# frosinastojanovska/image-captioning

Hardware: AMD Instinct MI355X
Metric: captions/sec (train step) on 1024px x 32RoI x 15tok synth (higher is better)
Workload: dtype f32 (split-bf16x3 products, fp32 accumulate: 73 of 85 conv layers on the bf16 pipe, the rest and the decoder exact fp32 MFMA); 1 GPU; BASELINE configs[2] (configs[3] at 8 GPUs): frozen ResNet-101+FPN fwd + PyramidROIAlign + RoI head + v2-inject decoder fwd/bwd + AMSGrad, 1024x1024 synth images, 32 RoI/img, 15-token captions, V=10000; backbone=resnet101, images_per_gpu=2, global_batch_images=2, parallelism=dp1, stage4_blocks=22, pipeline=encoder(i+1) || decoder(i), 2 HIP streams, rccl_ranks=1

## Files before the change

image-captioning_amd/_lib.py:

```python
import ctypes as C
import os

_HERE = os.path.dirname(os.path.abspath(__file__))
LIB_PATH = os.path.join(_HERE, "csrc", "libdcap_hip.so")

c_float_p = C.POINTER(C.c_float)
c_int32_p = C.POINTER(C.c_int32)
c_uint8_p = C.POINTER(C.c_uint8)


class GemmDesc(C.Structure):
    _fields_ = [("M", C.c_int), ("N", C.c_int), ("K", C.c_int),
                ("A", C.c_void_p), ("lda", C.c_int), ("a_trans", C.c_int),
                ("a_gather", C.c_void_p),
                ("B", C.c_void_p), ("ldb", C.c_int), ("b_trans", C.c_int),
                ("C", C.c_void_p), ("ldc", C.c_int),
                ("scale", C.c_void_p), ("shift", C.c_void_p),
                ("residual", C.c_void_p), ("ldr", C.c_int), ("res_rows", C.c_int),
                ("relu", C.c_int), ("accumulate", C.c_int), ("split_k", C.c_int)]


class GemmBf16Desc(C.Structure):
    _fields_ = [("M", C.c_int), ("N", C.c_int), ("K", C.c_int),
                ("A", C.c_void_p), ("lda", C.c_int), ("a_trans", C.c_int),
# ... 169 lines not shown


class DetectionTargetsDesc(C.Structure):
    _fields_ = [("n_proposals", C.c_int), ("n_gt", C.c_int), ("n_rois", C.c_int), ("T", C.c_int),
                ("proposals", C.c_void_p), ("gt_boxes", C.c_void_p), ("gt_captions", C.c_void_p),
                ("max_positive", C.c_int), ("inv_ratio", C.c_float), ("shuffle", C.c_int),
                ("seed", C.c_uint32), ("offset", C.c_uint32), ("offset_dev", C.c_void_p),
                ("rois", C.c_void_p), ("captions", C.c_void_p), ("counts", C.c_void_p)]


class PwChainDesc(C.Structure):
    _fields_ = [("M", C.c_int), ("K1", C.c_int), ("N1", C.c_int), ("N2", C.c_int),
                ("x", C.c_void_p), ("w1", C.c_void_p), ("scale1", C.c_void_p), ("shift1", C.c_void_p), ("residual", C.c_void_p),
                ("relu1", C.c_int), ("y", C.c_void_p), ("w2", C.c_void_p), ("scale2", C.c_void_p), ("shift2", C.c_void_p),
                ("relu2", C.c_int), ("z", C.c_void_p), ("w1_b3", C.c_void_p), ("w2_b3", C.c_void_p)]


class RegSegments(C.Structure):
    _fields_ = [("start", C.c_void_p), ("coef", C.c_void_p), ("mask", C.c_void_p), ("nseg", C.c_int)]


class AmsgradDesc(C.Structure):
    _fields_ = [("n", C.c_size_t), ("p", C.c_void_p), ("g", C.c_void_p), ("m", C.c_void_p),
                ("v", C.c_void_p), ("vhat", C.c_void_p),
                ("lr_t", C.c_float), ("beta1", C.c_float), ("beta2", C.c_float), ("eps", C.c_float),
                ("grad_scale", C.c_float), ("gnorm_sq", C.c_void_p), ("clipnorm", C.c_float),
                ("p_bf16", C.c_void_p), ("n_bf16", C.c_size_t), ("lr_t_dev", C.c_void_p), ("reg", C.POINTER(RegSegments))]


SYMBOLS = {
# ... 13 lines not shown
    "dc_cast_f32_bf16": (C.c_int, [C.c_void_p, C.c_void_p, C.c_size_t, C.c_void_p]),
    "dc_cast_bf16_f32": (C.c_int, [C.c_void_p, C.c_void_p, C.c_size_t, C.c_void_p]),
    "dc_cast_f32_bf16_2d": (C.c_int, [C.c_void_p, C.c_int, C.c_void_p, C.c_int, C.c_int, C.c_int, C.c_int, C.c_void_p]),
    "dc_split_bf16x3_f32": (C.c_int, [C.c_void_p, C.c_void_p, C.c_size_t, C.c_void_p]),
    "dc_conv2d_workspace_bytes": (C.c_size_t, [C.POINTER(ConvDesc)]),
    "dc_conv2d_nhwc_f32": (C.c_int, [C.POINTER(ConvDesc), C.c_void_p, C.c_size_t, C.c_void_p]),
    "dc_conv2d_tile_config": (C.c_int, [C.POINTER(ConvDesc), C.POINTER(C.c_int), C.POINTER(C.c_int), C.POINTER(C.c_int)]),
    "dc_conv2d_is_pointwise": (C.c_int, [C.POINTER(ConvDesc)]),
    "dc_conv2d_winograd_weight_bytes": (C.c_size_t, [C.c_int, C.c_int]),
    "dc_conv2d_winograd_pack_f32": (C.c_int, [C.c_void_p, C.c_void_p, C.c_int, C.c_int, C.c_void_p]),
    "dc_pw_chain_supported": (C.c_int, [C.c_int, C.c_int, C.c_int]),
    "dc_pw_chain_pack_f32": (C.c_int, [C.c_void_p, C.c_void_p, C.c_int, C.c_int, C.c_void_p]),
    "dc_pw_chain_pack_b3": (C.c_int, [C.c_void_p, C.c_void_p, C.c_int, C.c_int, C.c_void_p]),
    "dc_pw_chain_f32": (C.c_int, [C.POINTER(PwChainDesc), C.c_void_p]),
    "dc_pw_chain_kernel_name": (C.c_int, [C.POINTER(PwChainDesc), C.c_char_p, C.c_size_t]),
    "dc_conv2d_winograd_b3_weight_bytes": (C.c_size_t, [C.c_int, C.c_int]),
    "dc_conv2d_winograd_pack_b3": (C.c_int, [C.c_void_p, C.c_void_p, C.c_int, C.c_int, C.c_void_p]),
    "dc_conv2d_kernel_name": (C.c_int, [C.POINTER(ConvDesc), C.c_char_p, C.c_size_t]),
    "dc_conv2d_wgrad_workspace_bytes": (C.c_size_t, [C.POINTER(ConvDesc)]),
    "dc_conv2d_wgrad_f32": (C.c_int, [C.POINTER(ConvDesc), C.c_void_p, C.c_size_t, C.c_void_p]),
    "dc_roi_align_pyramid_bwd_f32": (C.c_int, [C.POINTER(RoiAlignDesc), C.c_void_p]),
    "dc_downsample2x_sum_f32": (C.c_int, [C.c_void_p, C.c_void_p, C.c_int, C.c_int, C.c_int, C.c_int, C.c_int, C.c_void_p]),
    "dc_downsample2x_sum_dual_f32": (C.c_int, [C.c_void_p, C.c_void_p, C.c_void_p, C.c_int, C.c_int, C.c_int, C.c_int, C.c_int, C.c_void_p]),
    "dc_maxpool2x2s2_f32": (C.c_int, [C.c_void_p, C.c_void_p, C.c_int, C.c_int, C.c_int, C.c_int, C.c_void_p]),
    "dc_maxpool3x3s2_same_f32": (C.c_int, [C.c_void_p, C.c_void_p, C.c_int, C.c_int, C.c_int, C.c_int, C.c_void_p]),
    "dc_mold_image_padded_f32": (C.c_int, [C.c_void_p, C.c_void_p, C.c_int, C.c_int, C.c_int, C.c_int, C.c_float, C.c_float, C.c_float, C.c_void_p]),
    "dc_mold_image_rgbx_f32": (C.c_int, [C.c_void_p, C.c_void_p, C.c_int, C.c_int, C.c_int,
                                         C.c_float, C.c_float, C.c_float, C.c_void_p]),
    "dc_roi_align_pyramid_f32": (C.c_int, [C.POINTER(RoiAlignDesc), C.c_void_p]),
    "dc_roi_tile_groups": (C.c_int, [C.POINTER(RoiGroupsDesc), C.c_void_p]),
# ... 102 lines not shown
```

image-captioning_amd/csrc/conv_chain.hip:

```cpp
#include "igemm_bf16s.h"
#include <algorithm>

namespace dcap {
namespace chain {

struct Args {
    const float* x;
    const f4* w1;
    const float* scale1;
    const float* shift1;
    const float* residual;
    float* y;
    const f4* w2;
    const float* scale2;
    const float* shift2;
    float* z;
    int M, K1, relu1, relu2;
    unsigned w1_bytes, w2_bytes;
};

__global__ void chain_pack_kernel(const float* __restrict__ w, float* __restrict__ out, int N, int K) {
    const long total = (long)N * K;
    const int NG = K >> 3;
    for (long idx = (long)blockIdx.x * blockDim.x + threadIdx.x; idx < total; idx += (long)gridDim.x * blockDim.x) {
        const int cout = (int)(idx / K), k = (int)(idx - (long)cout * K);
        const int cb = cout >> 5, i = cout & 31, g = k >> 3, h = (k >> 2) & 1, e = k & 3;
        out[(((long)cb * NG + g) * 64 + (h * 32 + i)) * 4 + e] = w[idx];
    }
}

__global__ void chain_pack_b3_kernel(const float* __restrict__ w, unsigned short* __restrict__ out, int N, int K) {
    const long total = (long)N * K;
    const int NG = K >> 4;
// ... 222 lines not shown
    }
    }
    if (m0 + p < a.M) {
#pragma unroll
        for (int gq = 0; gq < 4; ++gq) {
            const int c0 = wave * 32 + 8 * gq + 4 * h;
            f4 v = {acc2[4 * gq], acc2[4 * gq + 1], acc2[4 * gq + 2], acc2[4 * gq + 3]};
            if (a.scale2) v = v * *reinterpret_cast<const f4*>(a.scale2 + c0);
            v = v + *reinterpret_cast<const f4*>(a.shift2 + c0);
            if (a.relu2) v = f4{fmaxf(v[0], 0.f), fmaxf(v[1], 0.f), fmaxf(v[2], 0.f), fmaxf(v[3], 0.f)};
            *reinterpret_cast<f4*>(a.z + (long)(m0 + p) * N2 + c0) = v;
        }
    }
}

template <int K1, int N1, int N2>
__global__ __launch_bounds__(512, 1) void pw_chain_stream_kernel(Args a) {
    extern __shared__ __attribute__((aligned(16))) float smem[];
    constexpr int LDW1 = K1 + 4, LDW2 = N1 + 4, KH = K1 / 2, NG1 = K1 / 8, NG2 = N1 / 8;
    float* const W1s = smem;
    float* const W2s = W1s + N1 * LDW1;
    float* const sc1 = W2s + N2 * LDW2;
    float* const sh1 = sc1 + N1;
    float* const sc2 = sh1 + N1;
    float* const sh2 = sc2 + N2;
    const int tid = threadIdx.x, lane = tid & 63, wave = tid >> 6;
    const int i = lane & 31, h = lane >> 5;
    for (int idx = tid; idx < N1 * (K1 / 4); idx += 512) {
        const int c = idx / (K1 / 4), k4 = idx - c * (K1 / 4);
        *reinterpret_cast<f4*>(&W1s[c * LDW1 + 4 * k4]) = a.w1[((c >> 5) * NG1 + (k4 >> 1)) * 64 + 32 * (k4 & 1) + (c & 31)];
    }
    for (int idx = tid; idx < N2 * (N1 / 4); idx += 512) {
        const int c = idx / (N1 / 4), k4 = idx - c * (N1 / 4);
        *reinterpret_cast<f4*>(&W2s[c * LDW2 + 4 * k4]) = a.w2[((c >> 5) * NG2 + (k4 >> 1)) * 64 + 32 * (k4 & 1) + (c & 31)];
    }
    for (int c = tid; c < N1; c += 512) {
        sc1[c] = a.scale1 ? a.scale1[c] : 1.f;
        sh1[c] = a.shift1[c];
    }
    for (int c = tid; c < N2; c += 512) {
        sc2[c] = a.scale2 ? a.scale2[c] : 1.f;
        sh2[c] = a.shift2[c];
    }
    __syncthreads();
    const int strips = (a.M + 31) / 32;
    for (int st = blockIdx.x * 8 + wave; st < strips; st += gridDim.x * 8) {
        const int prow = st * 32 + i;
        const bool pv = prow < a.M;
        const int p = min(prow, a.M - 1);
        const float* xr = a.x + (long)p * K1 + KH * h;
        f4 xs[KH / 4];
#pragma unroll
        for (int j = 0; j < KH / 4; ++j) xs[j] = *reinterpret_cast<const f4*>(xr + 4 * j);
        const float* rrow = a.residual ? a.residual + (long)p * N1 + 4 * h : nullptr;
        float* const yrow = a.y + (long)p * N1 + 4 * h;
        f32x16 acc2[N2 / 32];
#pragma unroll
        for (int nb = 0; nb < N2 / 32; ++nb)
#pragma unroll
            for (int r = 0; r < 16; ++r) acc2[nb][r] = 0.f;
        for (int cb = 0; cb < N1; cb += 64) {
            f4 r0[4], r1[4];
            if (rrow) {
#pragma unroll
                for (int q = 0; q < 4; ++q) {
                    r0[q] = *reinterpret_cast<const f4*>(rrow + cb + 8 * q);
                    r1[q] = *reinterpret_cast<const f4*>(rrow + cb + 32 + 8 * q);
                }
            }
            f32x16 acc0, acc1;
#pragma unroll
            for (int r = 0; r < 16; ++r) { acc0[r] = 0.f; acc1[r] = 0.f; }
            const float* wa0 = &W1s[(cb + i) * LDW1 + KH * h];
            const float* wa1 = wa0 + 32 * LDW1;
#pragma unroll
            for (int j = 0; j < KH / 4; ++j) {
                const f4 a0 = *reinterpret_cast<const f4*>(wa0 + 4 * j);
                const f4 a1 = *reinterpret_cast<const f4*>(wa1 + 4 * j);
                const f4 b = xs[j];
#pragma unroll
                for (int e = 0; e < 4; ++e) {
                    acc0 = __builtin_amdgcn_mfma_f32_32x32x2f32(a0[e], b[e], acc0, 0, 0, 0);
                    acc1 = __builtin_amdgcn_mfma_f32_32x32x2f32(a1[e], b[e], acc1, 0, 0, 0);
                }
            }
            f4 y0[4], y1[4];
#pragma unroll
            for (int q = 0; q < 4; ++q) {
                const int c0 = cb + 8 * q + 4 * h;
                f4 v0 = f4{acc0[4 * q], acc0[4 * q + 1], acc0[4 * q + 2], acc0[4 * q + 3]} * *reinterpret_cast<const f4*>(&sc1[c0]) + *reinterpret_cast<const f4*>(&sh1[c0]);
                f4 v1 = f4{acc1[4 * q], acc1[4 * q + 1], acc1[4 * q + 2], acc1[4 * q + 3]} * *reinterpret_cast<const f4*>(&sc1[c0 + 32]) +
                        *reinterpret_cast<const f4*>(&sh1[c0 + 32]);
                if (rrow) { v0 += r0[q]; v1 += r1[q]; }
                if (a.relu1) {
                    v0 = f4{fmaxf(v0[0], 0.f), fmaxf(v0[1], 0.f), fmaxf(v0[2], 0.f), fmaxf(v0[3], 0.f)};
                    v1 = f4{fmaxf(v1[0], 0.f), fmaxf(v1[1], 0.f), fmaxf(v1[2], 0.f), fmaxf(v1[3], 0.f)};
                }
                if (pv) {
                    *reinterpret_cast<f4*>(yrow + cb + 8 * q) = v0;
                    *reinterpret_cast<f4*>(yrow + cb + 32 + 8 * q) = v1;
                }
                y0[q] = v0;
                y1[q] = v1;
            }
#pragma unroll
            for (int q = 0; q < 4; ++q)
#pragma unroll
                for (int nb = 0; nb < N2 / 32; ++nb) {
                    const float* w2r = &W2s[(nb * 32 + i) * LDW2 + cb + 8 * q + 4 * h];
                    const f4 wa = *reinterpret_cast<const f4*>(w2r);
                    const f4 wb = *reinterpret_cast<const f4*>(w2r + 32);
#pragma unroll
                    for (int e = 0; e < 4; ++e) {
                        acc2[nb] = __builtin_amdgcn_mfma_f32_32x32x2f32(wa[e], y0[q][e], acc2[nb], 0, 0, 0);
                        acc2[nb] = __builtin_amdgcn_mfma_f32_32x32x2f32(wb[e], y1[q][e], acc2[nb], 0, 0, 0);
                    }
                }
        }
// ... 1 lines not shown
            float* const zrow = a.z + (long)p * N2 + 4 * h;
#pragma unroll
            for (int nb = 0; nb < N2 / 32; ++nb)
#pragma unroll
                for (int q = 0; q < 4; ++q) {
                    const int c0 = nb * 32 + 8 * q + 4 * h;
                    f4 v = f4{acc2[nb][4 * q], acc2[nb][4 * q + 1], acc2[nb][4 * q + 2], acc2[nb][4 * q + 3]} * *reinterpret_cast<const f4*>(&sc2[c0]) +
                           *reinterpret_cast<const f4*>(&sh2[c0]);
                    if (a.relu2) v = f4{fmaxf(v[0], 0.f), fmaxf(v[1], 0.f), fmaxf(v[2], 0.f), fmaxf(v[3], 0.f)};
                    *reinterpret_cast<f4*>(zrow + nb * 32 + 8 * q) = v;
                }
        }
    }
}

static int launch_stream_64_256_64(const Args& a, hipStream_t s) {
    constexpr int K1 = 64, N1 = 256, N2 = 64;
    constexpr size_t lds = ((size_t)N1 * (K1 + 4) + (size_t)N2 * (N1 + 4) + 2 * N1 + 2 * N2) * sizeof(float);
    DC_ENSURE_DYN_LDS((&pw_chain_stream_kernel<K1, N1, N2>), 160 * 1024);
    const int strips = (a.M + 31) / 32;
    const int grid = std::max(1, std::min(kNumCU, (strips + 7) / 8));
    hipLaunchKernelGGL((pw_chain_stream_kernel<K1, N1, N2>), dim3(grid), dim3(512), lds, s, a);
    return check_launch("pw_chain_stream_kernel");
}

template <int CB1, int NB2, bool B3>
static int launch(const Args& a, hipStream_t s) {
    constexpr size_t lds = (size_t)32 * (CB1 * 256 + 4) * sizeof(float);
    DC_ENSURE_DYN_LDS((&pw_chain_kernel<CB1, NB2, B3>), 160 * 1024);
    hipLaunchKernelGGL((pw_chain_kernel<CB1, NB2, B3>), dim3((a.M + 31) / 32), dim3(512), lds, s, a);
    return check_launch("pw_chain_kernel");
}

}
}

using namespace dcap;

// ... 28 lines not shown
extern "C" int dc_pw_chain_f32(const dc_pw_chain_desc* d, void* stream) {
    const bool b3 = d && d->w1_b3 && d->w2_b3;
    DC_REQUIRE(d && d->x && (b3 || (d->w1 && d->w2)) && d->shift1 && d->y && d->shift2 && d->z && d->M > 0, DC_EINVAL, "dc_pw_chain: bad arguments");
    DC_REQUIRE(dc_pw_chain_supported(d->K1, d->N1, d->N2), DC_EINVAL,
               "dc_pw_chain: (K1, N1, N2) = (%d, %d, %d) is not a covered shape (K1 %% 32 == 0; N1 -> N2 = 1024 -> 256 or 512 -> 128; or 64 -> 256 -> 64)", d->K1, d->N1, d->N2);
    DC_REQUIRE(d->N1 != 256 || !b3, DC_EINVAL, "dc_pw_chain: the 64 -> 256 -> 64 seam takes fp32 products (dc_pw_chain_pack_f32 weights)");
    DC_REQUIRE(aligned16(d->x) && aligned16(b3 ? (const void*)d->w1_b3 : (const void*)d->w1) && aligned16(b3 ? (const void*)d->w2_b3 : (const void*)d->w2) && aligned16(d->y) && aligned16(d->z) && aligned16(d->shift1) && aligned16(d->shift2) &&
                   (!d->scale1 || aligned16(d->scale1)) && (!d->scale2 || aligned16(d->scale2)) && (!d->residual || aligned16(d->residual)),
               DC_EALIGN, "dc_pw_chain: every pointer must be 16-byte aligned");
    chain::Args a;
    a.x = d->x; a.w1 = b3 ? reinterpret_cast<const f4*>(d->w1_b3) : reinterpret_cast<const f4*>(d->w1); a.scale1 = d->scale1; a.shift1 = d->shift1; a.residual = d->residual; a.y = d->y;
    a.w2 = b3 ? reinterpret_cast<const f4*>(d->w2_b3) : reinterpret_cast<const f4*>(d->w2); a.scale2 = d->scale2; a.shift2 = d->shift2; a.z = d->z;
    a.M = d->M; a.K1 = d->K1; a.relu1 = d->relu1; a.relu2 = d->relu2;
    a.w1_bytes = (unsigned)((size_t)d->N1 * d->K1 * (b3 ? 6 : 4));
    a.w2_bytes = (unsigned)((size_t)d->N2 * d->N1 * (b3 ? 6 : 4));
    hipStream_t s = static_cast<hipStream_t>(stream);
    if (d->N1 == 256) return chain::launch_stream_64_256_64(a, s);
    if (b3) return d->N1 == 1024 ? chain::launch<4, 8, true>(a, s) : chain::launch<2, 4, true>(a, s);
    return d->N1 == 1024 ? chain::launch<4, 8, false>(a, s) : chain::launch<2, 4, false>(a, s);
}
```

image-captioning_amd/encoder.py:

```python
import ctypes as C

import numpy as np
import torch

from . import _lib, ops, step_graph
from ._lib import ConvBf16Desc, ConvDesc, PwChainDesc, check
from .layers import ConvSpec, resnet_fpn_convs
from .packing import fold_bn, pack_conv_kernel, pack_stem_kernel


DEFAULT_CONV_MATH = "f32"


def conv_math_mode(math=None):
    import os
    name = math if math is not None else os.environ.get("DCAP_CONV_MATH", DEFAULT_CONV_MATH)
    try:
        return {"f32": _lib.MATH_F32, "bf16x3": _lib.MATH_BF16X3, "bf16x2": _lib.MATH_BF16X2, "bf16": _lib.MATH_BF16}[name]
    except KeyError:
        raise ValueError("conv math must be 'f32', 'bf16x3', 'bf16x2' or 'bf16', got %r" % (name,))


def conv_math_name(mode):
    return {_lib.MATH_F32: "f32", _lib.MATH_BF16X3: "bf16x3", _lib.MATH_BF16X2: "bf16x2", _lib.MATH_BF16: "bf16"}.get(mode, str(mode))
# ... 5 lines not shown
    pad = (channels or k.shape[3]) - k.shape[3]
    if pad < 0:
        raise ValueError("rpn head needs %d channels, got %d" % (k.shape[3], channels))
    if pad:
        k = np.concatenate([k, np.zeros(k.shape[:3] + (pad,), np.float32)], axis=3)
        b = np.concatenate([b, np.zeros(pad, np.float32)])
    return k, b


class EncoderPlan:
    feat_channels = 256
    fast_bf16 = False

    def __init__(self, weights, batch, height, width, device, stage4_blocks=22,
                 mean_pixel=(123.7, 116.8, 103.9), use_graph=True, rpn=None, external=None, math=None, external_bn=None, train_stages=(),
                 winograd=None, wino_products=None, pw_chain=None, layer_math=None):
        if height % 64 or width % 64:
            raise ValueError("Image size must be dividable by 2 at least 6 times (got %dx%d)" % (height, width))
        self.lib = _lib.load()
        self.math = conv_math_mode(math)
        import os
        self.fast_bf16 = self.math == _lib.MATH_BF16
        self.winograd = (os.environ.get("DCAP_WINOGRAD", "1") != "0") if winograd is None else bool(winograd)
        self.wino_products = wino_products or os.environ.get("DCAP_WINO_PRODUCTS", "b3")
        if self.wino_products not in ("b3", "f32"):
            raise ValueError("wino_products must be 'b3' or 'f32'")
        self.pw_chain = (os.environ.get("DCAP_PW_CHAIN", "1") != "0") if pw_chain is None else bool(pw_chain)
        self.layer_math = (os.environ.get("DCAP_LAYER_MATH", "1") != "0") if layer_math is None else bool(layer_math)
        self._wchain = {}
        self._wwino = {}
        self._twin = {}
        self._wb = {}
        self.B, self.H, self.W = batch, height, width
        self.device = torch.device(device)
        self.mean_pixel = [float(v) for v in mean_pixel]
        self.stage4_blocks = stage4_blocks
        self.use_graph = bool(use_graph)
        self._steps = {}
        self._specs = {s.name: s for s in resnet_fpn_convs(stage4_blocks)}
        self.rpn = rpn
        self._external = dict(external or {})
        self._external_bn = dict(external_bn or {})
# ... 125 lines not shown
        if s.k != 1:
            return self.math
        if s.stride == 2 and s.cout >= 512 and s.cout > s.cin:
            return _lib.MATH_BF16X3
        if s.stride == 1 and 128 <= s.cin <= 512 and s.cout >= 256:
            return _lib.MATH_BF16X3
        return self.math

    def _chain_ok(self, name_c, name_a, mid, cout, pixels):
        sc, sa = self._specs[name_c], self._specs[name_a]
        if cout >= 512 and pixels < 32 * 192:
            return False
        return (self.pw_chain and self.math == _lib.MATH_F32 and not self.fast_bf16 and sc.k == 1 and sa.k == 1 and sc.stride == 1 and sa.stride == 1
                and name_c not in self._external and name_a not in self._external and ops.pw_chain_supported(mid, cout, mid))

    def _chain(self, name_c, x, y, residual, name_a, z):
        (w1, sc1, sh1), (w2, sc2, sh2) = self._w[name_c], self._w[name_a]
        b3 = self.wino_products == "b3" and x.shape[3] >= 128
        for n, w in ((name_c, w1), (name_a, w2)):
            if n not in self._wchain:
                self._wchain[n] = (ops.pw_chain_pack_b3 if b3 else ops.pw_chain_pack)(w)
        N, H, W, K1 = x.shape
        d = PwChainDesc()
        d.M, d.K1, d.N1, d.N2 = N * H * W, K1, y.shape[3], z.shape[3]
        d.x, d.shift1, d.y = x.data_ptr(), sh1.data_ptr(), y.data_ptr()
        if b3:
            d.w1_b3, d.w2_b3 = self._wchain[name_c].data_ptr(), self._wchain[name_a].data_ptr()
        else:
            d.w1, d.w2 = self._wchain[name_c].data_ptr(), self._wchain[name_a].data_ptr()
        d.scale1 = None if sc1 is None else sc1.data_ptr()
        d.residual = None if residual is None else residual.data_ptr()
        d.shift2, d.z = sh2.data_ptr(), z.data_ptr()
        d.scale2 = None if sc2 is None else sc2.data_ptr()
        d.relu1 = d.relu2 = 1
        self._ops.append(("chain", d, name_c + "+" + name_a))
        self.flops += 2.0 * d.M * (d.K1 * d.N1 + d.N1 * d.N2)

    def _build(self):
        B, H, W = self.B, self.H, self.W
        self._ops, self._ws_bytes, self.flops, self._bufs = [], 0, 0.0, []
        self._twin, self._wb = {}, {}
        self.images = torch.empty((B, H, W, 3), dtype=torch.uint8, device=self.device)
        rgbx = torch.empty((B, H, W, 4), dtype=torch.float32, device=self.device)
        for name, bnp in self._external_bn.items():
            _, sc, sh = self._external[name]
            self._ops.append(("bnfold", bnp, sc, sh))
        self._ops.append(("mold", self.images, rgbx))
        c1 = self._buf(H // 2, W // 2, 64)
        self._conv("conv1", rgbx, c1)
        x = self._buf(H // 4, W // 4, 64)
        self._ops.append(("pool", c1, x))
        if self.fast_bf16:
            self._ops.append(("cast", x, self._bf(x)))
        self.saved[1] = dict(rgbx=rgbx, c1=c1, pooled=x)

        def stage(s, blocks, mid, cout, stride, x):
            h, w = x.shape[1] // stride, x.shape[2] // stride
            keep = s in self.train_stages
            if not keep:
                m1, m2, sc = self._buf(h, w, mid), self._buf(h, w, mid), self._buf(h, w, cout)
                pp = [self._buf(h, w, cout), self._buf(h, w, cout)]
            final = self._buf(h, w, cout)
            self.saved[s] = []
            pending = None
            for i, blk in enumerate(blocks):
                cn = "res%d%s_branch" % (s, blk)
                if keep:
                    m1, m2 = self._buf(h, w, mid), self._buf(h, w, mid)
                    sc = self._buf(h, w, cout) if i == 0 else None
                    out = final if i == len(blocks) - 1 else self._buf(h, w, cout)
                    self.saved[s].append(dict(name=cn, x=x, m1=m1, m2=m2, sc=sc, out=out, stride=stride if i == 0 else 1))
                else:
                    out = final if i == len(blocks) - 1 else pp[i & 1]
                if pending is not None:
                    self._chain(pending[0], pending[1], x, pending[2], cn + "2a", m1)
                    pending = None
                else:
                    self._conv(cn + "2a", x, m1, f32=keep, bf16=True)
                self._conv(cn + "2b", m1, m2, f32=keep, bf16=True)
                res = x
                if i == 0:
                    self._conv(cn + "1", x, sc, relu=False)
                    res = sc
                nxt = "res%d%s_branch2a" % (s, blocks[i + 1]) if i + 1 < len(blocks) else None
                if nxt is not None and not keep and self._chain_ok(cn + "2c", nxt, mid, cout, x.shape[0] * m2.shape[1] * m2.shape[2]):
                    pending = (cn + "2c", m2, res)
                else:
                    self._conv(cn + "2c", m2, out, residual=res, res_mode=1, bf16=True)
                x = out
            return x

        C2 = stage(2, "abc", 64, 256, 1, x)
        C3 = stage(3, "abcd", 128, 512, 2, C2)
        C4 = stage(4, ["a"] + [chr(98 + i) for i in range(self.stage4_blocks)], 256, 1024, 2, C3)
        C5 = stage(5, "abc", 512, 2048, 2, C4)
        self.C = (C2, C3, C4, C5)
        self._n_trunk = len(self._ops)
        self.pre = None
        t5, t4 = self._buf(H // 32, W // 32, 256), self._buf(H // 16, W // 16, 256)
        t3, t2 = self._buf(H // 8, W // 8, 256), self._buf(H // 4, W // 4, 256)
        self._conv("fpn_c5p5", C5, t5, relu=False, bf16=True)
# ... 47 lines not shown

    def _run_ops(self, lo=0, hi=None):
        lib = self.lib
        stream = C.c_void_p(torch.cuda.current_stream().cuda_stream)
        wsp, wsb = C.c_void_p(self._ws.data_ptr()), self._ws.numel()
        for op in self._ops[lo:hi]:
            kind = op[0]
            if kind == "conv":
                rc = lib.dc_conv2d_nhwc_f32(C.byref(op[1]), wsp, wsb, stream)
                if rc:
                    check(rc, "dc_conv2d_nhwc_f32(%s)" % op[2])
            elif kind == "chain":
                rc = lib.dc_pw_chain_f32(C.byref(op[1]), stream)
                if rc:
                    check(rc, "dc_pw_chain_f32(%s)" % op[2])
            elif kind == "bconv":
                rc = lib.dc_conv2d_bf16(C.byref(op[1]), wsp, wsb, stream)
                if rc:
                    check(rc, "dc_conv2d_bf16(%s)" % op[2])
            elif kind == "cast":
                ops.to_bf16(op[1], out=op[2])
            elif kind == "bnfold":
                b = op[1]
                ops.bn_fold(b["gamma"], b["beta"], b["bias"], b["mean"], b["var"], op[2], op[3])
            elif kind == "mold":
                ops.mold_image_rgbx(op[1], self.mean_pixel, out=op[2])
            elif kind == "sub2":
                ops.subsample2(op[1], out=op[2])
            else:
                ops.maxpool3x3s2_same(op[1], out=op[2])

    def conv_table(self):
        rows = []
        for op in self._ops:
            if op[0] == "chain":
                d, buf = op[1], C.create_string_buffer(64)
                check(self.lib.dc_pw_chain_kernel_name(C.byref(d), buf, 64), "dc_pw_chain_kernel_name")
                rows.append((op[2], 2.0 * d.M * (d.K1 * d.N1 + d.N1 * d.N2), 32, d.N1, 1, buf.value.decode()))
                continue
            if op[0] != "conv":
                continue
            d, bm, bn, sk = op[1], C.c_int(), C.c_int(), C.c_int()
            check(self.lib.dc_conv2d_tile_config(C.byref(d), C.byref(bm), C.byref(bn), C.byref(sk)), "dc_conv2d_tile_config")
            buf = C.create_string_buffer(128)
            check(self.lib.dc_conv2d_kernel_name(C.byref(d), buf, 128), "dc_conv2d_kernel_name")
            s = self._specs[op[2]]
            rows.append((op[2], 2.0 * d.N * d.Ho * d.Wo * d.Cout * s.k * s.k * s.cin, bm.value, bn.value, sk.value, buf.value.decode()))
        return rows

    def conv_algorithmic_bytes(self):
        out = {}
        for op in self._ops:
            if op[0] == "chain":
                d = op[1]
                out[op[2]] = 4.0 * (d.M * (d.K1 + (2 if d.residual else 1) * d.N1 + d.N2) + d.K1 * d.N1 + d.N1 * d.N2)
                continue
            if op[0] != "conv":
                continue
            d, s = op[1], self._specs[op[2]]
            wbytes = ((16 * (6 if self.wino_products == "b3" else 4)) if op[2] in self._wwino else s.k * s.k * 4) * d.Cin * s.cout
            b = 4.0 * d.N * d.H * d.W * d.Cin + 4.0 * d.N * d.Ho * d.Wo * d.Cout + wbytes
            if d.res_mode == 1:
                b += 4.0 * d.N * d.Ho * d.Wo * d.Cout
            elif d.res_mode == 2:
                b += 1.0 * d.N * d.Ho * d.Wo * d.Cout
            out[op[2]] = b
        return out

    def time_convs(self, reps=3, beside=None):
        lib = self.lib
        stream = C.c_void_p(torch.cuda.current_stream().cuda_stream)
        wsp, wsb = C.c_void_p(self._ws.data_ptr()), self._ws.numel()
        convs = [op for op in self._ops if op[0] in ("conv", "chain")]
        acc = [0.0] * len(convs)
        for _ in range(reps):
            self._run_ops()
            torch.cuda.synchronize()
            if beside is not None:
                beside()
            evs = []
            for op in convs:
                e0, e1 = torch.cuda.Event(enable_timing=True), torch.cuda.Event(enable_timing=True)
                e0.record()
                rc = lib.dc_pw_chain_f32(C.byref(op[1]), stream) if op[0] == "chain" else lib.dc_conv2d_nhwc_f32(C.byref(op[1]), wsp, wsb, stream)
                e1.record()
                if rc:
                    check(rc, "dc_conv2d_nhwc_f32(%s)" % op[2])
                evs.append((e0, e1))
            torch.cuda.synchronize()
            for i, (e0, e1) in enumerate(evs):
                acc[i] += e0.elapsed_time(e1)
        return [(op[2], a / reps) for op, a in zip(convs, acc)]

    def time_bconvs(self, reps=3):
        lib = self.lib
        stream = C.c_void_p(torch.cuda.current_stream().cuda_stream)
        wsp, wsb = C.c_void_p(self._ws.data_ptr()), self._ws.numel()
        convs = [op for op in self._ops if op[0] == "bconv"]
        acc = [0.0] * len(convs)
# ... 191 lines not shown
```

image-captioning_amd/ops.py:

```python
import contextlib
import ctypes as C
import os

import numpy as np

import torch

from . import _lib
from ._lib import (PwChainDesc, ConvBf16Desc, AmsgradDesc, DetectionTargetsDesc, BnReluDesc, ConvDesc, ConvWgradBf16Desc, GemmBf16Desc, VocabCeDesc, ProposalDesc, RpnLossDesc, GemmDesc, LstmBwdDesc, LstmFwdDesc, RoiAlignDesc, RoiGroupsDesc,
                   SoftmaxCeDesc, VocabTop1Desc, VocabTopkDesc, VocabTop1Bf16Desc, VocabTopkBf16Desc, VocabSampleDesc, VocabSampleBf16Desc, BeamSelectDesc, BeamStepDesc, LstmStepDesc, RefineDesc, check)


def _stream():
    return C.c_void_p(torch.cuda.current_stream().cuda_stream)


def _ptr(t):
    return None if t is None else C.c_void_p(t.data_ptr())


def _chk(t, dtype=torch.float32, name="tensor"):
    if not t.is_cuda:
        raise _lib.DcapError("%s must live on the GPU (no CPU path exists)" % name)
    if t.dtype != dtype:
# ... 254 lines not shown
        if not t.is_contiguous():
            raise _lib.DcapError("pw_chain: tensors must be contiguous")
    d = PwChainDesc()
    d.M, d.K1, d.N1, d.N2 = M, K1, N1, N2
    d.x, d.shift1, d.y = _chk(x, name="x").data_ptr(), _chk(shift1, name="shift1").data_ptr(), _chk(y, name="y").data_ptr()
    d.shift2, d.z = _chk(shift2, name="shift2").data_ptr(), _chk(z, name="z").data_ptr()
    if b3:
        d.w1_b3, d.w2_b3 = _chk(w1f, torch.int16, "w1").data_ptr(), _chk(w2f, torch.int16, "w2").data_ptr()
    else:
        d.w1, d.w2 = _chk(w1f, name="w1").data_ptr(), _chk(w2f, name="w2").data_ptr()
    d.scale1 = None if scale1 is None else _chk(scale1, name="scale1").data_ptr()
    d.scale2 = None if scale2 is None else _chk(scale2, name="scale2").data_ptr()
    d.residual = None if residual is None else _chk(residual, name="residual").data_ptr()
    d.relu1, d.relu2 = int(relu1), int(relu2)
    check(lib.dc_pw_chain_f32(C.byref(d), _stream()), "dc_pw_chain_f32")
    return y, z


def winograd_pack_b3(w_packed, cin, cout, out=None):
    lib = _lib.load()
    _chk(w_packed, name="w")
    if not w_packed.is_contiguous() or w_packed.numel() != 9 * cin * cout:
        raise _lib.DcapError("winograd_pack_b3: w must be the contiguous packed 3x3 kernel [Cout, 9*Cin]")
    nbytes = lib.dc_conv2d_winograd_b3_weight_bytes(cin, cout)
    if nbytes == 0:
        raise _lib.DcapError("winograd_pack_b3: Cin and Cout must be multiples of 32")
    if out is None:
        out = torch.empty((nbytes // 2,), dtype=torch.int16, device=w_packed.device)
    check(lib.dc_conv2d_winograd_pack_b3(_ptr(w_packed), _ptr(out), cin, cout, _stream()), "dc_conv2d_winograd_pack_b3")
    return out
# ... 1115 lines not shown
```

include/dcap.h:

```cpp
#ifndef DCAP_H
#define DCAP_H

#include <stddef.h>
#include <stdint.h>

#ifdef __cplusplus
extern "C" {
#endif

#define DC_OK            0
#define DC_EINVAL       -1
#define DC_EALIGN       -2
#define DC_EWORKSPACE   -3
#define DC_ELAUNCH      -4

#define DC_ABI_VERSION 600
int         dc_version(void);
const char* dc_last_error(void);

typedef struct {
    int M, N, K;
    const float*   A;  int lda;  int a_trans;
    const int32_t* a_gather;
    const float*   B;  int ldb;  int b_trans;
// ... 110 lines not shown
    int relu1;
    float* y;
    const float* w2;
    const float* scale2;
    const float* shift2;
    int relu2;
    float* z;
    const uint16_t* w1_b3;
    const uint16_t* w2_b3;
} dc_pw_chain_desc;
int dc_pw_chain_supported(int K1, int N1, int N2);
int dc_pw_chain_pack_f32(const float* w, float* out, int N, int K, void* stream);
int dc_pw_chain_pack_b3(const float* w, uint16_t* out, int N, int K, void* stream);
int dc_pw_chain_f32(const dc_pw_chain_desc* d, void* stream);
int dc_pw_chain_kernel_name(const dc_pw_chain_desc* d, char* buf, size_t buf_bytes);

int    dc_set_persistent_cus(int n);
int    dc_get_persistent_cus(void);

size_t dc_conv2d_wgrad_workspace_bytes(const dc_conv_desc* d);
int    dc_conv2d_wgrad_f32(const dc_conv_desc* d, void* workspace, size_t workspace_bytes, void* stream);

int dc_maxpool3x3s2_same_f32(const float* x, float* y, int N, int H, int W, int C, void* stream);

int dc_maxpool2x2s2_f32(const float* x, float* y, int N, int H, int W, int C, void* stream);

int dc_mold_image_rgbx_f32(const uint8_t* img, float* out, int N, int H, int W,
                           float mean_r, float mean_g, float mean_b, void* stream);
int dc_mold_image_padded_f32(const uint8_t* img, float* out, int N, int H, int W, int channels,
                             float mean_r, float mean_g, float mean_b, void* stream);
// ... 406 lines not shown
```

Baseline: 12970 captions/s.

## Fuse stage-1 projection shortcut conv into the pointwise chain kernel

Adds a variant of the 64->256->64 streaming pointwise chain kernel that also computes the first block's 1x1 projection shortcut from x in registers, instead of running a separate conv and reading its output back as the residual. The shortcut weights are streamed per column block through a buffer resource, and the encoder build now skips allocating and launching the separate shortcut conv when the shapes match. This saves one kernel launch and a full write and read of the 256-channel shortcut tensor, at the cost of more registers and MFMA work inside the fused kernel, which runs with one block per CU.

```diff
diff --git a/image-captioning_amd/_lib.py b/image-captioning_amd/_lib.py
--- a/image-captioning_amd/_lib.py
+++ b/image-captioning_amd/_lib.py
@@ -207,6 +207,10 @@
                 ("x", C.c_void_p), ("w1", C.c_void_p), ("scale1", C.c_void_p), ("shift1", C.c_void_p), ("residual", C.c_void_p),
                 ("relu1", C.c_int), ("y", C.c_void_p), ("w2", C.c_void_p), ("scale2", C.c_void_p), ("shift2", C.c_void_p),
                 ("relu2", C.c_int), ("z", C.c_void_p), ("w1_b3", C.c_void_p), ("w2_b3", C.c_void_p)]
+
+
+class PwChainScDesc(C.Structure):
+    _fields_ = [("chain", PwChainDesc), ("xs", C.c_void_p), ("wp", C.c_void_p), ("scale_p", C.c_void_p), ("shift_p", C.c_void_p)]
 
 
 class RegSegments(C.Structure):
@@ -250,6 +254,9 @@
     "dc_pw_chain_pack_b3": (C.c_int, [C.c_void_p, C.c_void_p, C.c_int, C.c_int, C.c_void_p]),
     "dc_pw_chain_f32": (C.c_int, [C.POINTER(PwChainDesc), C.c_void_p]),
     "dc_pw_chain_kernel_name": (C.c_int, [C.POINTER(PwChainDesc), C.c_char_p, C.c_size_t]),
+    "dc_pw_chain_sc_supported": (C.c_int, [C.c_int, C.c_int, C.c_int]),
+    "dc_pw_chain_sc_f32": (C.c_int, [C.POINTER(PwChainScDesc), C.c_void_p]),
+    "dc_pw_chain_sc_kernel_name": (C.c_int, [C.POINTER(PwChainScDesc), C.c_char_p, C.c_size_t]),
     "dc_conv2d_winograd_b3_weight_bytes": (C.c_size_t, [C.c_int, C.c_int]),
     "dc_conv2d_winograd_pack_b3": (C.c_int, [C.c_void_p, C.c_void_p, C.c_int, C.c_int, C.c_void_p]),
     "dc_conv2d_kernel_name": (C.c_int, [C.POINTER(ConvDesc), C.c_char_p, C.c_size_t]),
diff --git a/image-captioning_amd/csrc/conv_chain.hip b/image-captioning_amd/csrc/conv_chain.hip
--- a/image-captioning_amd/csrc/conv_chain.hip
+++ b/image-captioning_amd/csrc/conv_chain.hip
@@ -17,6 +17,10 @@
     float* z;
     int M, K1, relu1, relu2;
     unsigned w1_bytes, w2_bytes;
+    const float* xsc;
+    const f4* wp;
+    const float* scale_p;
+    const float* shift_p;
 };
 
 __global__ void chain_pack_kernel(const float* __restrict__ w, float* __restrict__ out, int N, int K) {
@@ -269,8 +273,8 @@
     }
 }
 
-template <int K1, int N1, int N2>
-__global__ __launch_bounds__(512, 1) void pw_chain_stream_kernel(Args a) {
+template <int K1, int N1, int N2, bool SC>
+__device__ __forceinline__ void chain_stream_body(const Args& a) {
     extern __shared__ __attribute__((aligned(16))) float smem[];
     constexpr int LDW1 = K1 + 4, LDW2 = N1 + 4, KH = K1 / 2, NG1 = K1 / 8, NG2 = N1 / 8;
     float* const W1s = smem;
@@ -279,6 +283,8 @@
     float* const sh1 = sc1 + N1;
     float* const sc2 = sh1 + N1;
     float* const sh2 = sc2 + N2;
+    float* const scp = sh2 + N2;
+    float* const shp = scp + N1;
     const int tid = threadIdx.x, lane = tid & 63, wave = tid >> 6;
     const int i = lane & 31, h = lane >> 5;
     for (int idx = tid; idx < N1 * (K1 / 4); idx += 512) {
@@ -296,6 +302,25 @@
     for (int c = tid; c < N2; c += 512) {
         sc2[c] = a.scale2 ? a.scale2[c] : 1.f;
         sh2[c] = a.shift2[c];
+    }
+    f4 wp0[KH / 4], wp1[KH / 4];
+    const unsigned wp_lane = (unsigned)((KH / 8 * h * 64 + i) * 16);
+    [[maybe_unused]] __amdgpu_buffer_rsrc_t rsrcp;
+    [[maybe_unused]] auto ldwp = [&](int cb) {
+#pragma unroll
+        for (int j = 0; j < KH / 4; ++j) {
+            const unsigned so = (unsigned)((((cb >> 5) * NG1 + (j >> 1)) * 64 + 32 * (j & 1)) * 16);
+            wp0[j] = buf_f4s(rsrcp, wp_lane, so);
+            wp1[j] = buf_f4s(rsrcp, wp_lane, so + (unsigned)(NG1 * 1024));
+        }
+    };
+    if constexpr (SC) {
+        for (int c = tid; c < N1; c += 512) {
+            scp[c] = a.scale_p ? a.scale_p[c] : 1.f;
+            shp[c] = a.shift_p[c];
+        }
+        rsrcp = __builtin_amdgcn_make_buffer_rsrc(const_cast<f4*>(a.wp), 0, N1 * K1 * 4, 0x00020000);
+        ldwp(0);
     }
     __syncthreads();
     const int strips = (a.M + 31) / 32;
@@ -307,7 +332,13 @@
         f4 xs[KH / 4];
 #pragma unroll
         for (int j = 0; j < KH / 4; ++j) xs[j] = *reinterpret_cast<const f4*>(xr + 4 * j);
-        const float* rrow = a.residual ? a.residual + (long)p * N1 + 4 * h : nullptr;
+        f4 xp[KH / 4];
+        if constexpr (SC) {
+            const float* xpr = a.xsc + (long)p * K1 + KH * h;
+#pragma unroll
+            for (int j = 0; j < KH / 4; ++j) xp[j] = *reinterpret_cast<const f4*>(xpr + 4 * j);
+        }
+        const float* rrow = (!SC && a.residual) ? a.residual + (long)p * N1 + 4 * h : nullptr;
         float* const yrow = a.y + (long)p * N1 + 4 * h;
         f32x16 acc2[N2 / 32];
 #pragma unroll
@@ -322,6 +353,21 @@
                     r0[q] = *reinterpret_cast<const f4*>(rrow + cb + 8 * q);
                     r1[q] = *reinterpret_cast<const f4*>(rrow + cb + 32 + 8 * q);
                 }
+            }
+            f32x16 accp0, accp1;
+            if constexpr (SC) {
+#pragma unroll
+                for (int r = 0; r < 16; ++r) { accp0[r] = 0.f; accp1[r] = 0.f; }
+#pragma unroll
+                for (int j = 0; j < KH / 4; ++j) {
+                    const f4 b = xp[j];
+#pragma unroll
+                    for (int e = 0; e < 4; ++e) {
+                        accp0 = __builtin_amdgcn_mfma_f32_32x32x2f32(wp0[j][e], b[e], accp0, 0, 0, 0);
+                        accp1 = __builtin_amdgcn_mfma_f32_32x32x2f32(wp1[j][e], b[e], accp1, 0, 0, 0);
+                    }
+                }
+                __builtin_amdgcn_sched_barrier(0);
             }
             f32x16 acc0, acc1;
 #pragma unroll
@@ -347,6 +393,13 @@
                 f4 v1 = f4{acc1[4 * q], acc1[4 * q + 1], acc1[4 * q + 2], acc1[4 * q + 3]} * *reinterpret_cast<const f4*>(&sc1[c0 + 32]) +
                         *reinterpret_cast<const f4*>(&sh1[c0 + 32]);
                 if (rrow) { v0 += r0[q]; v1 += r1[q]; }
+                if constexpr (SC) {
+                    const f4 u0 = f4{accp0[4 * q], accp0[4 * q + 1], accp0[4 * q + 2], accp0[4 * q + 3]} * *reinterpret_cast<const f4*>(&scp[c0]) + *reinterpret_cast<const f4*>(&shp[c0]);
+                    const f4 u1 = f4{accp1[4 * q], accp1[4 * q + 1], accp1[4 * q + 2], accp1[4 * q + 3]} * *reinterpret_cast<const f4*>(&scp[c0 + 32]) +
+                                  *reinterpret_cast<const f4*>(&shp[c0 + 32]);
+                    v0 += u0;
+                    v1 += u1;
+                }
                 if (a.relu1) {
                     v0 = f4{fmaxf(v0[0], 0.f), fmaxf(v0[1], 0.f), fmaxf(v0[2], 0.f), fmaxf(v0[3], 0.f)};
                     v1 = f4{fmaxf(v1[0], 0.f), fmaxf(v1[1], 0.f), fmaxf(v1[2], 0.f), fmaxf(v1[3], 0.f)};
@@ -357,6 +410,11 @@
                 }
                 y0[q] = v0;
                 y1[q] = v1;
+            }
+            if constexpr (SC) {
+                __builtin_amdgcn_sched_barrier(0);
+                ldwp((cb + 64) & (N1 - 1));
+                __builtin_amdgcn_sched_barrier(0);
             }
 #pragma unroll
             for (int q = 0; q < 4; ++q)
@@ -388,14 +446,30 @@
     }
 }
 
+template <int K1, int N1, int N2>
+__global__ __launch_bounds__(512, 1) void pw_chain_stream_kernel(Args a) {
+    chain_stream_body<K1, N1, N2, false>(a);
+}
+template <int K1, int N1, int N2>
+__global__ __launch_bounds__(512, 1) void pw_chain_stream_sc_kernel(Args a) {
+    chain_stream_body<K1, N1, N2, true>(a);
+}
+
+template <bool SC>
 static int launch_stream_64_256_64(const Args& a, hipStream_t s) {
     constexpr int K1 = 64, N1 = 256, N2 = 64;
-    constexpr size_t lds = ((size_t)N1 * (K1 + 4) + (size_t)N2 * (N1 + 4) + 2 * N1 + 2 * N2) * sizeof(float);
-    DC_ENSURE_DYN_LDS((&pw_chain_stream_kernel<K1, N1, N2>), 160 * 1024);
+    constexpr size_t lds = ((size_t)N1 * (K1 + 4) + (size_t)N2 * (N1 + 4) + (SC ? 4 : 2) * N1 + 2 * N2) * sizeof(float);
     const int strips = (a.M + 31) / 32;
     const int grid = std::max(1, std::min(kNumCU, (strips + 7) / 8));
-    hipLaunchKernelGGL((pw_chain_stream_kernel<K1, N1, N2>), dim3(grid), dim3(512), lds, s, a);
-    return check_launch("pw_chain_stream_kernel");
+    if constexpr (SC) {
+        DC_ENSURE_DYN_LDS((&pw_chain_stream_sc_kernel<K1, N1, N2>), 160 * 1024);
+        hipLaunchKernelGGL((pw_chain_stream_sc_kernel<K1, N1, N2>), dim3(grid), dim3(512), lds, s, a);
+        return check_launch("pw_chain_stream_sc_kernel");
+    } else {
+        DC_ENSURE_DYN_LDS((&pw_chain_stream_kernel<K1, N1, N2>), 160 * 1024);
+        hipLaunchKernelGGL((pw_chain_stream_kernel<K1, N1, N2>), dim3(grid), dim3(512), lds, s, a);
+        return check_launch("pw_chain_stream_kernel");
+    }
 }
 
 template <int CB1, int NB2, bool B3>
@@ -454,8 +528,38 @@
     a.M = d->M; a.K1 = d->K1; a.relu1 = d->relu1; a.relu2 = d->relu2;
     a.w1_bytes = (unsigned)((size_t)d->N1 * d->K1 * (b3 ? 6 : 4));
     a.w2_bytes = (unsigned)((size_t)d->N2 * d->N1 * (b3 ? 6 : 4));
+    a.xsc = nullptr; a.wp = nullptr; a.scale_p = nullptr; a.shift_p = nullptr;
     hipStream_t s = static_cast<hipStream_t>(stream);
-    if (d->N1 == 256) return chain::launch_stream_64_256_64(a, s);
+    if (d->N1 == 256) return chain::launch_stream_64_256_64<false>(a, s);
     if (b3) return d->N1 == 1024 ? chain::launch<4, 8, true>(a, s) : chain::launch<2, 4, true>(a, s);
     return d->N1 == 1024 ? chain::launch<4, 8, false>(a, s) : chain::launch<2, 4, false>(a, s);
 }
+
+extern "C" int dc_pw_chain_sc_supported(int K1, int N1, int N2) { return (K1 == 64 && N1 == 256 && N2 == 64) ? 1 : 0; }
+
+extern "C" int dc_pw_chain_sc_kernel_name(const dc_pw_chain_sc_desc* d, char* buf, size_t buf_bytes) {
+    DC_REQUIRE(d && buf && buf_bytes >= 48, DC_EINVAL, "dc_pw_chain_sc_kernel_name: bad arguments");
+    snprintf(buf, buf_bytes, "pw_chain_stream_sc_kernel<%d, %d, %d>", d->chain.K1, d->chain.N1, d->chain.N2);
+    return DC_OK;
+}
+
+extern "C" int dc_pw_chain_sc_f32(const dc_pw_chain_sc_desc* d, void* stream) {
+    DC_REQUIRE(d, DC_EINVAL, "dc_pw_chain_sc: bad arguments");
+    const dc_pw_chain_desc& c = d->chain;
+    DC_REQUIRE(c.x && c.w1 && c.w2 && c.shift1 && c.y && c.shift2 && c.z && d->xs && d->wp && d->shift_p && c.M > 0, DC_EINVAL, "dc_pw_chain_sc: bad arguments");
+    DC_REQUIRE(dc_pw_chain_sc_supported(c.K1, c.N1, c.N2), DC_EINVAL, "dc_pw_chain_sc: (K1, N1, N2) = (%d, %d, %d) is not a covered shape (64 -> 256 -> 64)", c.K1, c.N1,
+               c.N2);
+    DC_REQUIRE(!c.w1_b3 && !c.w2_b3, DC_EINVAL, "dc_pw_chain_sc: fp32 products only (dc_pw_chain_pack_f32 weights; w1_b3 / w2_b3 must be NULL)");
+    DC_REQUIRE(!c.residual, DC_EINVAL, "dc_pw_chain_sc: the shortcut is computed from x; residual must be NULL");
+    DC_REQUIRE(aligned16(c.x) && aligned16(d->xs) && aligned16(c.w1) && aligned16(c.w2) && aligned16(d->wp) && aligned16(c.y) && aligned16(c.z) && aligned16(c.shift1) && aligned16(c.shift2) &&
+                   aligned16(d->shift_p) && (!c.scale1 || aligned16(c.scale1)) && (!c.scale2 || aligned16(c.scale2)) && (!d->scale_p || aligned16(d->scale_p)),
+               DC_EALIGN, "dc_pw_chain_sc: every pointer must be 16-byte aligned");
+    chain::Args a;
+    a.x = c.x; a.w1 = reinterpret_cast<const f4*>(c.w1); a.scale1 = c.scale1; a.shift1 = c.shift1; a.residual = nullptr; a.y = c.y;
+    a.w2 = reinterpret_cast<const f4*>(c.w2); a.scale2 = c.scale2; a.shift2 = c.shift2; a.z = c.z;
+    a.M = c.M; a.K1 = c.K1; a.relu1 = c.relu1; a.relu2 = c.relu2;
+    a.w1_bytes = (unsigned)((size_t)c.N1 * c.K1 * 4);
+    a.w2_bytes = (unsigned)((size_t)c.N2 * c.N1 * 4);
+    a.xsc = d->xs; a.wp = reinterpret_cast<const f4*>(d->wp); a.scale_p = d->scale_p; a.shift_p = d->shift_p;
+    return chain::launch_stream_64_256_64<true>(a, static_cast<hipStream_t>(stream));
+}
diff --git a/image-captioning_amd/encoder.py b/image-captioning_amd/encoder.py
--- a/image-captioning_amd/encoder.py
+++ b/image-captioning_amd/encoder.py
@@ -4,7 +4,7 @@
 import torch
 
 from . import _lib, ops, step_graph
-from ._lib import ConvBf16Desc, ConvDesc, PwChainDesc, check
+from ._lib import ConvBf16Desc, ConvDesc, PwChainDesc, PwChainScDesc, check
 from .layers import ConvSpec, resnet_fpn_convs
 from .packing import fold_bn, pack_conv_kernel, pack_stem_kernel
 
@@ -43,7 +43,7 @@
 
     def __init__(self, weights, batch, height, width, device, stage4_blocks=22,
                  mean_pixel=(123.7, 116.8, 103.9), use_graph=True, rpn=None, external=None, math=None, external_bn=None, train_stages=(),
-                 winograd=None, wino_products=None, pw_chain=None, layer_math=None):
+                 winograd=None, wino_products=None, pw_chain=None, layer_math=None, sc_chain=None):
         if height % 64 or width % 64:
             raise ValueError("Image size must be dividable by 2 at least 6 times (got %dx%d)" % (height, width))
         self.lib = _lib.load()
@@ -55,6 +55,7 @@
         if self.wino_products not in ("b3", "f32"):
             raise ValueError("wino_products must be 'b3' or 'f32'")
         self.pw_chain = (os.environ.get("DCAP_PW_CHAIN", "1") != "0") if pw_chain is None else bool(pw_chain)
+        self.sc_chain = (os.environ.get("DCAP_SC_CHAIN", "1") != "0") if sc_chain is None else bool(sc_chain)
         self.layer_math = (os.environ.get("DCAP_LAYER_MATH", "1") != "0") if layer_math is None else bool(layer_math)
         self._wchain = {}
         self._wwino = {}
@@ -210,14 +211,15 @@
         return (self.pw_chain and self.math == _lib.MATH_F32 and not self.fast_bf16 and sc.k == 1 and sa.k == 1 and sc.stride == 1 and sa.stride == 1
                 and name_c not in self._external and name_a not in self._external and ops.pw_chain_supported(mid, cout, mid))
 
-    def _chain(self, name_c, x, y, residual, name_a, z):
+    def _chain(self, name_c, x, y, residual, name_a, z, proj=None):
         (w1, sc1, sh1), (w2, sc2, sh2) = self._w[name_c], self._w[name_a]
         b3 = self.wino_products == "b3" and x.shape[3] >= 128
-        for n, w in ((name_c, w1), (name_a, w2)):
+        for n, w in ((name_c, w1), (name_a, w2)) + (((proj[0], self._w[proj[0]][0]),) if proj else ()):
             if n not in self._wchain:
                 self._wchain[n] = (ops.pw_chain_pack_b3 if b3 else ops.pw_chain_pack)(w)
         N, H, W, K1 = x.shape
-        d = PwChainDesc()
+        ds = PwChainScDesc() if proj else None
+        d = ds.chain if proj else PwChainDesc()
         d.M, d.K1, d.N1, d.N2 = N * H * W, K1, y.shape[3], z.shape[3]
         d.x, d.shift1, d.y = x.data_ptr(), sh1.data_ptr(), y.data_ptr()
         if b3:
@@ -229,7 +231,14 @@
         d.shift2, d.z = sh2.data_ptr(), z.data_ptr()
         d.scale2 = None if sc2 is None else sc2.data_ptr()
         d.relu1 = d.relu2 = 1
-        self._ops.append(("chain", d, name_c + "+" + name_a))
+        if proj:
+            wp, scp, shp = self._w[proj[0]]
+            ds.xs, ds.wp, ds.shift_p = proj[1].data_ptr(), self._wchain[proj[0]].data_ptr(), shp.data_ptr()
+            ds.scale_p = None if scp is None else scp.data_ptr()
+            self._ops.append(("scchain", ds, name_c + "+" + proj[0] + "+" + name_a))
+            self.flops += 2.0 * d.M * d.K1 * d.N1
+        else:
+            self._ops.append(("chain", d, name_c + "+" + name_a))
         self.flops += 2.0 * d.M * (d.K1 * d.N1 + d.N1 * d.N2)
 
     def _build(self):
@@ -254,7 +263,7 @@
             h, w = x.shape[1] // stride, x.shape[2] // stride
             keep = s in self.train_stages
             if not keep:
-                m1, m2, sc = self._buf(h, w, mid), self._buf(h, w, mid), self._buf(h, w, cout)
+                m1, m2 = self._buf(h, w, mid), self._buf(h, w, mid)
                 pp = [self._buf(h, w, cout), self._buf(h, w, cout)]
             final = self._buf(h, w, cout)
             self.saved[s] = []
@@ -269,18 +278,25 @@
                 else:
                     out = final if i == len(blocks) - 1 else pp[i & 1]
                 if pending is not None:
-                    self._chain(pending[0], pending[1], x, pending[2], cn + "2a", m1)
+                    self._chain(pending[0], pending[1], x, pending[2], cn + "2a", m1, *pending[3:])
                     pending = None
                 else:
                     self._conv(cn + "2a", x, m1, f32=keep, bf16=True)
                 self._conv(cn + "2b", m1, m2, f32=keep, bf16=True)
+                nxt = "res%d%s_branch2a" % (s, blocks[i + 1]) if i + 1 < len(blocks) else None
+                chained = nxt is not None and not keep and self._chain_ok(cn + "2c", nxt, mid, cout, x.shape[0] * m2.shape[1] * m2.shape[2])
                 res = x
                 if i == 0:
-                    self._conv(cn + "1", x, sc, relu=False)
-                    res = sc
-                nxt = "res%d%s_branch2a" % (s, blocks[i + 1]) if i + 1 < len(blocks) else None
-                if nxt is not None and not keep and self._chain_ok(cn + "2c", nxt, mid, cout, x.shape[0] * m2.shape[1] * m2.shape[2]):
-                    pending = (cn + "2c", m2, res)
+                    if (chained and stride == 1 and self.sc_chain and cn + "1" not in self._external and x.shape[3] == mid and
+                            ops.pw_chain_sc_supported(mid, cout, mid)):
+                        res = None
+                    else:
+                        if not keep:
+                            sc = self._buf(h, w, cout)
+                        self._conv(cn + "1", x, sc, relu=False)
+                        res = sc
+                if chained:
+                    pending = (cn + "2c", m2, res) if res is not None else (cn + "2c", m2, None, (cn + "1", x))
                 else:
                     self._conv(cn + "2c", m2, out, residual=res, res_mode=1, bf16=True)
                 x = out
@@ -358,6 +374,10 @@
                 rc = lib.dc_pw_chain_f32(C.byref(op[1]), stream)
                 if rc:
                     check(rc, "dc_pw_chain_f32(%s)" % op[2])
+            elif kind == "scchain":
+                rc = lib.dc_pw_chain_sc_f32(C.byref(op[1]), stream)
+                if rc:
+                    check(rc, "dc_pw_chain_sc_f32(%s)" % op[2])
             elif kind == "bconv":
                 rc = lib.dc_conv2d_bf16(C.byref(op[1]), wsp, wsb, stream)
                 if rc:
@@ -382,6 +402,11 @@
                 check(self.lib.dc_pw_chain_kernel_name(C.byref(d), buf, 64), "dc_pw_chain_kernel_name")
                 rows.append((op[2], 2.0 * d.M * (d.K1 * d.N1 + d.N1 * d.N2), 32, d.N1, 1, buf.value.decode()))
                 continue
+            if op[0] == "scchain":
+                d, buf = op[1].chain, C.create_string_buffer(64)
+                check(self.lib.dc_pw_chain_sc_kernel_name(C.byref(op[1]), buf, 64), "dc_pw_chain_sc_kernel_name")
+                rows.append((op[2], 2.0 * d.M * (2 * d.K1 * d.N1 + d.N1 * d.N2), 32, d.N1, 1, buf.value.decode()))
+                continue
             if op[0] != "conv":
                 continue
             d, bm, bn, sk = op[1], C.c_int(), C.c_int(), C.c_int()
@@ -398,6 +423,10 @@
             if op[0] == "chain":
                 d = op[1]
                 out[op[2]] = 4.0 * (d.M * (d.K1 + (2 if d.residual else 1) * d.N1 + d.N2) + d.K1 * d.N1 + d.N1 * d.N2)
+                continue
+            if op[0] == "scchain":
+                d = op[1].chain
+                out[op[2]] = 4.0 * (d.M * (2 * d.K1 + d.N1 + d.N2) + 2 * d.K1 * d.N1 + d.N1 * d.N2)
                 continue
             if op[0] != "conv":
                 continue
@@ -415,7 +444,7 @@
         lib = self.lib
         stream = C.c_void_p(torch.cuda.current_stream().cuda_stream)
         wsp, wsb = C.c_void_p(self._ws.data_ptr()), self._ws.numel()
-        convs = [op for op in self._ops if op[0] in ("conv", "chain")]
+        convs = [op for op in self._ops if op[0] in ("conv", "chain", "scchain")]
         acc = [0.0] * len(convs)
         for _ in range(reps):
             self._run_ops()
@@ -426,7 +455,10 @@
             for op in convs:
                 e0, e1 = torch.cuda.Event(enable_timing=True), torch.cuda.Event(enable_timing=True)
                 e0.record()
-                rc = lib.dc_pw_chain_f32(C.byref(op[1]), stream) if op[0] == "chain" else lib.dc_conv2d_nhwc_f32(C.byref(op[1]), wsp, wsb, stream)
+                if op[0] == "conv":
+                    rc = lib.dc_conv2d_nhwc_f32(C.byref(op[1]), wsp, wsb, stream)
+                else:
+                    rc = (lib.dc_pw_chain_f32 if op[0] == "chain" else lib.dc_pw_chain_sc_f32)(C.byref(op[1]), stream)
                 e1.record()
                 if rc:
                     check(rc, "dc_conv2d_nhwc_f32(%s)" % op[2])
diff --git a/image-captioning_amd/ops.py b/image-captioning_amd/ops.py
--- a/image-captioning_amd/ops.py
+++ b/image-captioning_amd/ops.py
@@ -7,7 +7,7 @@
 import torch
 
 from . import _lib
-from ._lib import (PwChainDesc, ConvBf16Desc, AmsgradDesc, DetectionTargetsDesc, BnReluDesc, ConvDesc, ConvWgradBf16Desc, GemmBf16Desc, VocabCeDesc, ProposalDesc, RpnLossDesc, GemmDesc, LstmBwdDesc, LstmFwdDesc, RoiAlignDesc, RoiGroupsDesc,
+from ._lib import (PwChainDesc, PwChainScDesc, ConvBf16Desc, AmsgradDesc, DetectionTargetsDesc, BnReluDesc, ConvDesc, ConvWgradBf16Desc, GemmBf16Desc, VocabCeDesc, ProposalDesc, RpnLossDesc, GemmDesc, LstmBwdDesc, LstmFwdDesc, RoiAlignDesc, RoiGroupsDesc,
                    SoftmaxCeDesc, VocabTop1Desc, VocabTopkDesc, VocabTop1Bf16Desc, VocabTopkBf16Desc, VocabSampleDesc, VocabSampleBf16Desc, BeamSelectDesc, BeamStepDesc, LstmStepDesc, RefineDesc, check)
 
 
@@ -292,6 +292,40 @@
     d.residual = None if residual is None else _chk(residual, name="residual").data_ptr()
     d.relu1, d.relu2 = int(relu1), int(relu2)
     check(lib.dc_pw_chain_f32(C.byref(d), _stream()), "dc_pw_chain_f32")
+    return y, z
+
+
+def pw_chain_sc_supported(k1, n1, n2):
+    return bool(_lib.load().dc_pw_chain_sc_supported(int(k1), int(n1), int(n2)))
+
+
+def pw_chain_sc(x, w1f, shift1, xs, wpf, shift_p, w2f, shift2, scale1=None, scale_p=None, scale2=None, relu1=True, relu2=True, y=None, z=None):
+    lib = _lib.load()
+    K1 = x.shape[-1]
+    M = x.numel() // K1
+    N1, N2 = w1f.shape[0], w2f.shape[0]
+    if tuple(xs.shape) != tuple(x.shape) or tuple(w1f.shape) != (N1, K1) or tuple(wpf.shape) != (N1, K1) or tuple(w2f.shape) != (N2, N1):
+        raise _lib.DcapError("pw_chain_sc: shapes do not chain: x %s, xs %s, w1 %s, wp %s, w2 %s" %
+                             (tuple(x.shape), tuple(xs.shape), tuple(w1f.shape), tuple(wpf.shape), tuple(w2f.shape)))
+    if y is None:
+        y = torch.empty(tuple(x.shape[:-1]) + (N1,), dtype=torch.float32, device=x.device)
+    if z is None:
+        z = torch.empty(tuple(x.shape[:-1]) + (N2,), dtype=torch.float32, device=x.device)
+    for t in (x, xs, y, z):
+        if not t.is_contiguous():
+            raise _lib.DcapError("pw_chain_sc: tensors must be contiguous")
+    d = PwChainScDesc()
+    c = d.chain
+    c.M, c.K1, c.N1, c.N2 = M, K1, N1, N2
+    c.x, c.shift1, c.y = _chk(x, name="x").data_ptr(), _chk(shift1, name="shift1").data_ptr(), _chk(y, name="y").data_ptr()
+    c.shift2, c.z = _chk(shift2, name="shift2").data_ptr(), _chk(z, name="z").data_ptr()
+    c.w1, c.w2 = _chk(w1f, name="w1").data_ptr(), _chk(w2f, name="w2").data_ptr()
+    c.scale1 = None if scale1 is None else _chk(scale1, name="scale1").data_ptr()
+    c.scale2 = None if scale2 is None else _chk(scale2, name="scale2").data_ptr()
+    c.relu1, c.relu2 = int(relu1), int(relu2)
+    d.xs, d.wp, d.shift_p = _chk(xs, name="xs").data_ptr(), _chk(wpf, name="wp").data_ptr(), _chk(shift_p, name="shift_p").data_ptr()
+    d.scale_p = None if scale_p is None else _chk(scale_p, name="scale_p").data_ptr()
+    check(lib.dc_pw_chain_sc_f32(C.byref(d), _stream()), "dc_pw_chain_sc_f32")
     return y, z
 
 
diff --git a/include/dcap.h b/include/dcap.h
--- a/include/dcap.h
+++ b/include/dcap.h
@@ -148,6 +148,16 @@
 int dc_pw_chain_pack_b3(const float* w, uint16_t* out, int N, int K, void* stream);
 int dc_pw_chain_f32(const dc_pw_chain_desc* d, void* stream);
 int dc_pw_chain_kernel_name(const dc_pw_chain_desc* d, char* buf, size_t buf_bytes);
+typedef struct {
+    dc_pw_chain_desc chain;
+    const float* xs;
+    const float* wp;
+    const float* scale_p;
+    const float* shift_p;
+} dc_pw_chain_sc_desc;
+int dc_pw_chain_sc_supported(int K1, int N1, int N2);
+int dc_pw_chain_sc_f32(const dc_pw_chain_sc_desc* d, void* stream);
+int dc_pw_chain_sc_kernel_name(const dc_pw_chain_sc_desc* d, char* buf, size_t buf_bytes);
 
 int    dc_set_persistent_cus(int n);
 int    dc_get_persistent_cus(void);
```

Result: no change. 12980 captions/s (median of 3 runs) (+0.1%).
